# junghan0611/node-replication

Measured on AMD Instinct MI355X. Metric: Mops/s whole node, NrHashMap 10% writes, 1/2/4/8 GPUs; replay HBM GB/s vs peak, higher is better.
Workload: dtype u64; 1 GPU; NrHashMap replica per GPU: 2^26-slot table, uniform keys over 10000000, prefill [0,8388608)->k+1, rounds of 1000000 ops/GPU = 100000 Put + 900000 Get; ops_per_gpu_per_round=1000000, put_responses=Ok(None) as benches/hashmap.rs:114-119, parallelism=replicas1

## Files before the change

### include/nrgpu_testing.h

```cpp
#ifndef NRGPU_TESTING_H
#define NRGPU_TESTING_H
#include "nrgpu.h"
#ifdef __cplusplus
extern "C" {
#endif
int nrg_test_sort_pairs(nrg_ctx* ctx, const uint32_t* d_keys, const uint32_t* d_vals, uint64_t n,
                        int key_bits, uint32_t* d_out_keys, uint32_t* d_out_vals);
int nrg_test_maxscan(nrg_ctx* ctx, const uint32_t* d_keys, const uint32_t* d_vals, uint64_t n,
                     uint32_t* d_out);
int nrg_test_lds_add_order(nrg_ctx* ctx, uint32_t keys, uint32_t trials, uint32_t blocks, uint64_t out[2]);
int nrg_test_ring_read(nrg_ctx* ctx, uint64_t phys, void* out);
int nrg_test_debug_read(nrg_ctx* ctx, uint64_t* out, uint64_t words);
int nrg_test_vspace_table(nrg_ctx* ctx, uint64_t table, uint64_t out[512]);
#define NRG_MF_PREAD_TILE 16384u

#define NRG_KNOB_STAMP_MAX 1
#define NRG_KNOB_SKEW_EVERY 2
#define NRG_KNOB_EPOCH_LIMIT 3
#define NRG_KNOB_K1 4
#define NRG_KNOB_EXP 6
#define NRG_KNOB_SY_SORT 7
#define NRG_KNOB_PIPELINE 8
#define NRG_KNOB_SY_FUSED 18
#define NRG_KNOB_COMB_SPIN 10
#define NRG_KNOB_COMB_DEPTH 11
#define NRG_KNOB_PA_TPB 16
#define NRG_KNOB_COMB_GATHER 15
#define NRG_KNOB_COMB_SERVE 17
#define NRG_KNOB_SMALL_MAX 12
#define NRG_KNOB_PART 13
#define NRG_KNOB_STALL 14
#define NRG_KNOB_SL_DELTA_MAX 20
int nrg_test_set_knob(nrg_ctx* ctx, int knob, uint64_t value);
int nrg_test_combiner_probe(nrg_combiner* m, uint64_t out[8]);
int nrg_test_combiner_times(nrg_combiner* m, uint64_t out[4]);

int nrg_test_loopback_collectives(int on);
int nrg_test_hm_skewed(nrg_ctx* ctx, int* out);
#ifdef __cplusplus
}
#endif
#endif
```

### node-replication_amd/csrc/hashmap.hip

```cpp
#include <cstring>

#include "internal.hpp"
#include "../../include/nrgpu_testing.h"

namespace nrg {

typedef u64 u64x2 __attribute__((ext_vector_type(2)));

template <typename T>
__device__ __forceinline__ void st_out(T* p, T v, bool plain) {
    if (plain) *p = v;
    else __builtin_nontemporal_store(v, p);
}
__device__ __forceinline__ void st_rec(nrg_put* p, const nrg_put& r, bool plain) {
    if (plain) *p = r;
    else __builtin_nontemporal_store(u64x2{r.key, r.val}, (u64x2*)p);
}

constexpr u64 PA_NT_MAX = 2000000;
template <bool NT, typename T>
__device__ __forceinline__ void st_pol(T* p, T v) {
    if constexpr (NT) __builtin_nontemporal_store(v, p);
    else *p = v;
}
// ... 308 lines not shown
#pragma unroll
    for (int q = 0; q < K1; q++) {
        const u64 i = base + (u64)q * TPB + threadIdx.x;
        if (i >= j.n) continue;
        const u64 k = rec[q].key;
        if (k == EMPTY_KEY) {
            if (ld_relaxed32(&ctl->sp_claim) == 0 && atomicCAS(&ctl->sp_claim, 0u, 1u) == 0u) {
                ctl->sp.st[(e - 1) & 1] = stamp_make(e, 0);
                created++;
            }
            atomicMax(&s_side, (u32)(i + 1));
            j.put_slot[i] = SIDE_SLOT;
            continue;
        }
        const long long s = find_or_claim_marked(table, k, home[q], tmask, key0[q], e, &created);
        if (s < 0) {
            atomicOr(&ctl->err, ERR_TABLE_FULL);
            j.put_slot[i] = FULL_SLOT;
            continue;
        }
        j.put_slot[i] = (u32)s;
        u32 h = (u32)(mix64((u64)s) & (HT - 1));
        for (;;) {
            const u32 old = atomicCAS(&s_slot[h], 0xFFFFFFFFu, (u32)s);
            if (old == 0xFFFFFFFFu || old == (u32)s) {
                dup += old == (u32)s ? 1u : 0u;
                break;
            }
            h = (h + 1) & (HT - 1);
        }
        atomicMax(&s_max[h], (u32)(i + 1));
    }
    if (created) atomicAdd(&s_created, created);
    if (dup) atomicAdd(&s_dup, dup);
    __syncthreads();
    for (int q = threadIdx.x; q < HT; q += TPB) {
        const u32 sl = s_slot[q];
        if (sl != 0xFFFFFFFFu) {
            const u64 mine = stamp_make(e, s_max[q]);
            const u64 old = atomicMax((unsigned long long*)&table[sl].st[par], (unsigned long long)mine);
            if (old < mine) {
                j.win[s_max[q] - 1] = e;
                if (stamp_epoch(old) == e && (u32)old) j.over[(u32)old - 1] = e;
            }
        }
    }
    if (threadIdx.x == 0) {
        if (s_side) atomicMax((unsigned long long*)&ctl->sp.st[par], (unsigned long long)stamp_make(e, s_side));
        if (s_created) atomicAdd(&j.created_acc[blk % HM_CREATED_SLOTS], (u64)s_created);
        if (s_dup && j.dup_acc) atomicAdd(&j.dup_acc[blk % HM_DUP_SLOTS], (u64)s_dup);
    }
}

__device__ __forceinline__ void apply_role(const ApplyJob& j, u32 blk, Slot* table, DevCtl* ctl) {
    const u64 i = (u64)blk * TPB + threadIdx.x;
    if (i >= j.n) return;
    const u32 par = j.epoch & 1;
    const u32 s = j.put_slot[i];
    const u64 want = stamp_make(j.epoch, i + 1);
    if (s == SIDE_SLOT) {
        if (ctl->sp.st[par] == want) ctl->sp.val = j.rec.at(i).val;
    } else if (s != FULL_SLOT) {
        if (j.win[i] == j.epoch && j.over[i] != j.epoch) __builtin_nontemporal_store(j.rec.at(i).val, &table[s].val);
    }
}

__device__ __forceinline__ bool resolve(u64 val, u64 st, const ReadJob& j, u64* v) {
    const u32 se = stamp_epoch(st);
    if (st == 0 || se > j.epoch) return false;
    *v = (se == j.epoch && j.use_rec) ? j.rec.at((u32)st - 1).val : val;
    return true;
}

constexpr int RPT = 1;
static_assert(RPT == 1, "read_role gives a wave 64 consecutive Gets");

__device__ __forceinline__ u32 quad_x1(u32 x) { return (u32)__builtin_amdgcn_update_dpp(0, (int)x, 0xB1, 0xF, 0xF, true); }
__device__ __forceinline__ u32 quad_x2(u32 x) { return (u32)__builtin_amdgcn_update_dpp(0, (int)x, 0x4E, 0xF, 0xF, true); }
__device__ __forceinline__ u64 quad_or(u64 x) {
    u32 lo = (u32)x, hi = (u32)(x >> 32);
    lo |= quad_x1(lo);
    hi |= quad_x1(hi);
    lo |= quad_x2(lo);
    hi |= quad_x2(hi);
    return ((u64)hi << 32) | lo;
}

constexpr int READ_PASSES = 4;
static_assert(READ_PASSES * 16 == 64, "a wave's passes of 16 quads cover its 64 Gets");
template <bool STAMP>
__device__ __forceinline__ void read_role(const ReadJob& j, u32 blk, const Slot* table, u32 shift, u64 tmask,
                                          const DevCtl* ctl) {
    const u32 par = j.epoch & 1;
    const auto quiet = [&] { return STAMP ? false : j.quiet; };
    const auto plain = [&] { return STAMP ? true : j.plain; };
    const u32 lane = lane_id(), sub = lane & 3, quad = lane >> 2, qsh = lane & ~3u;
    const u64 wbase = (u64)blk * TPB + (threadIdx.x & ~63u);
    if (wbase >= j.R) return;
    u64 k[READ_PASSES], s[READ_PASSES], st[READ_PASSES];
    u64x2 w[READ_PASSES];
#pragma unroll
    for (int p = 0; p < READ_PASSES; p++) {
        const u64 q = wbase + p * 16 + quad;
        k[p] = q < j.R ? j.keys[q] : EMPTY_KEY;
    }
#pragma unroll
// ... 14 lines not shown
        asm volatile("" : "+v"(kk), "+v"(vv), "+v"(stt));
        bool f = false, act = k[p] != EMPTY_KEY;
        for (u64 g = 0;; g++) {
            const bool hit = act && kk == k[p];
            if (hit) {
                if (quiet()) {
                    f = true;
                    v = vv;
                } else {
                    f = resolve(vv, stt, j, &v);
                }
            }
            const u64 done = __ballot(hit || !act || kk == EMPTY_KEY);
            act = ((done >> qsh) & 15) == 0 && g < (tmask >> 2);
            if (!__ballot(act)) break;
            if (act) {
                sl = (sl + 4) & tmask;
                const u64x2 x = *(const u64x2*)&table[sl];
                if (!quiet()) stt = table[sl].st[par];
                kk = x.x;
                vv = x.y;
            }
        }
        if (k[p] == EMPTY_KEY && sub == 0 && ctl->sp_claim) {
            if (quiet()) {
                f = true;
                v = ctl->sp.val;
            } else {
                f = resolve(ctl->sp.val, ctl->sp.st[par], j, &v);
            }
        }
        if (!f) v = 0;
        rv[p] = quad_or(v);
        fb[p] = __ballot(f);
    }
    u64 c = rv[0], b = fb[0];
#pragma unroll
    for (int p = 1; p < READ_PASSES; p++) {
        if (sub == (u32)p) c = rv[p];
        if ((lane >> 4) == (u32)p) b = fb[p];
    }
    const u64 v = __shfl(c, (int)(4 * (lane & 15) + (lane >> 4)), 64);
    const u64 q = wbase + lane;
    if (q < j.R) {
        st_out(&j.vals[q], v, plain());
        st_out(&j.found[q], (uint8_t)(((b >> (4 * (lane & 15))) & 15) != 0), plain());
    }
}

constexpr int IX_STAMP = 2;
constexpr int IX_PART = 3;
constexpr int IX_PART_ALL = 4;
constexpr int IX_PART_NODUP = 5;

template <int K1, int IX>
__global__ __launch_bounds__(TPB) __attribute__((amdgpu_num_sgpr(80))) void hm_round_kernel(IndexJob ij, StampJob sj,
                                                                                             ApplyJob aj, ReadJob rj,
                                                       Slot* table, u32 shift, u64 tmask, DevCtl* ctl) {
    extern __shared__ __attribute__((aligned(16))) char s_lds[];
    u32 b = blockIdx.x;
    if (rj.s_seq && b == gridDim.x - 1) {
        if (rj.s_seq && threadIdx.x < HM_DUP_SLOTS) {
            u64 v = atomicExch((unsigned long long*)&rj.s_acc[threadIdx.x], 0ull);
#pragma unroll
            for (int off = 32; off > 0; off >>= 1) v += __shfl_xor(v, off, 64);
            if (threadIdx.x == 0) {
                rj.s_host[1] = v;
                __threadfence_system();
                rj.s_host[0] = rj.s_seq;
            }
        }
        return;
    }
    const u32 nix = IX == IX_STAMP ? sj.nblocks : ij.nblocks;
    if (b < nix) {
        if constexpr (IX == IX_STAMP) stamp_index_role<K1>(sj, b, table, shift, tmask, ctl, s_lds);
        else part_role<K1, IX == IX_PART>(ij, b, shift, s_lds);
        return;
    }
    b -= nix;
    if (b < aj.nblocks) {
        apply_role(aj, b, table, ctl);
        return;
    }
    b -= aj.nblocks;
    read_role<IX == IX_STAMP>(rj, b, table, shift, tmask, ctl);
}

struct PApplyJob {
    const u64x2* ent;
    const u32* eidx;
    const u32* cnt;
    u32 ntiles, tile, nb;
    Slot* table;
    u32 shift;
    u64 tmask;
    DevCtl* ctl;
    u64* created_acc;
    u64 lo, resp_lo, resp_hi;
    u64* prev;
    uint8_t* prevf;
    u32 stall;
    u64* dbg;
};

template <bool PREV, int T>
struct PaGeo {
    static_assert(!PREV || T == 256, "previous values use 256-thread workgroups");
    static constexpr int TPB = T;
    static constexpr int C = PREV ? 512 : 4 * T;
    static constexpr int HT = 2 * C;
    static constexpr int PER = C / TPB;
    static constexpr u32 NB_LOG = T == 1024 ? 8 : T == 512 ? 9 : 10;
};

__device__ __forceinline__ u32 pa_hash(u64 k, u32 ht) { return (u32)(mix64(k) >> 40) & (ht - 1); }

template <int N, bool WANT_VAL>
__device__ __forceinline__ void pa_resolve(Slot* table, u32 shift, u64 tmask, const u64* k, const bool* on,
                                           long long* slot, bool* fresh, u64* val) {
    u64 s[N], kk[N], vv[N];
    u32 st[N];
#pragma unroll
    for (int r = 0; r < N; r++) {
        st[r] = on[r] ? 1u : 0u;
        s[r] = on[r] ? table_home(k[r], shift) : 0;
        slot[r] = -1;
        fresh[r] = false;
        kk[r] = EMPTY_KEY;
        vv[r] = 0;
        if (on[r]) {
            if (WANT_VAL) {
                const u64x2 x = *(const u64x2*)&table[s[r]];
                kk[r] = x.x;
                vv[r] = x.y;
            } else {
                kk[r] = ld_relaxed(&table[s[r]].key);
            }
        }
// ... 986 lines not shown
            ctl->sp.st[0] = ctl->sp.st[1] = STAMP_PRESENT;
            continue;
        }
        bool fresh;
        const long long s = claim_slot(table, r.x, table_home(r.x, shift), tmask, &fresh);
        if (s < 0) {
            atomicOr(&ctl->err, ERR_TABLE_FULL);
            continue;
        }
        table[s].val = r.y;
        table[s].st[0] = table[s].st[1] = STAMP_PRESENT;
        inserted += fresh;
    }
    if (inserted) atomicAdd(&s_ins, inserted);
    __syncthreads();
    if (threadIdx.x == 0 && s_ins) atomicAdd((unsigned long long*)&ctl->nkeys, (unsigned long long)s_ins);
}

struct SegArgs {
    u64 start[64];
    u64 total;
    u32 nseg;
    u32 words;
};

__global__ __launch_bounds__(TPB) void copy_segments_kernel(const u64* __restrict__ base, u64 seg_stride_words,
                                                            SegArgs a, u64* ring, u64 ring_mask, u64 dst_lo) {
    for (u64 r = blockIdx.x * (u64)TPB + threadIdx.x; r < a.total; r += (u64)gridDim.x * TPB) {
        u32 s = 0;
        while (s + 1 < a.nseg && a.start[s + 1] <= r) s++;
        const u64 j = r - a.start[s];
        const u64* srcp = base + s * seg_stride_words + j * a.words;
        u64* dst = ring + ((dst_lo + r) & ring_mask) * a.words;
        for (u32 q = 0; q < a.words; q++) dst[q] = srcp[q];
    }
}

static inline unsigned grid_for(u64 n, u64 cap = 4096) {
    u64 g = (n + TPB - 1) / TPB;
    if (g < 1) g = 1;
    if (g > cap) g = cap;
    return (unsigned)g;
}

static RecSrc ring_src(nrg_ctx* c, const nrg_put* src, u64 lo) {
    RecSrc r;
    r.src = src;
    r.ring = (const nrg_put*)c->d_ring;
    r.mask = c->log_size - 1;
    r.lo = lo;
    return r;
}

static u32 stamp_k1_for(const nrg_ctx* c, u64 n, u64 R) {
    if (c->hm.k1_items) return c->hm.k1_items >= 4 ? 4u : c->hm.k1_items >= 2 ? 2u : 1u;
    if (n <= (1u << 18)) return 1u;
    return n >= 655360 && R >= n ? 4u : 2u;
}

struct Launch {
    IndexJob ij{};
    StampJob sj{};
    ApplyJob aj{};
    ReadJob rj{};
    int ix = IX_PART_NODUP;
    u32 K1 = 1;
    u32 nb = 0;
};

static void attach_deferred(nrg_ctx* c, Launch& L) {
    const HmDeferred& p = c->hm.pend;
    L.rj.epoch = c->hm.epoch;
    if (p.valid) {
        const RecSrc rs = ring_src(c, p.src, p.lo);
        L.rj.keys = p.keys;
        L.rj.R = p.R;
        L.rj.vals = p.vals;
        L.rj.found = p.found;
        L.rj.epoch = p.epoch;
        L.rj.use_rec = p.apply;
        L.rj.rec = rs;
        if (p.apply) {
            L.aj.rec = rs;
            L.aj.n = p.n;
            L.aj.put_slot = c->hm.d_put_slot[p.epoch & 1];
            L.aj.win = L.aj.put_slot + c->hm.stamp_alloc;
            L.aj.over = L.aj.put_slot + 2 * c->hm.stamp_alloc;
            L.aj.epoch = p.epoch;
            L.aj.nblocks = (u32)((p.n + TPB - 1) / TPB);
        }
    }
    c->hm.pend = HmDeferred{};
}

template <int K1, int IX>
static void launch_round(nrg_ctx* c, const Launch& L, u32 blocks, unsigned lds) {
    NRG_LAUNCH(c, "hm_round", (hm_round_kernel<K1, IX>), blocks, TPB, lds, c->stream, L.ij, L.sj, L.aj, L.rj,
               c->hm.d_table, c->hm.slot_shift, (u64)(c->hm.slots - 1), c->d_ctl);
}

static hipError_t launch(nrg_ctx* c, Launch& L) {
    L.rj.nblocks = (u32)((L.rj.R + TPB * RPT - 1) / (TPB * RPT));
    const u32 nix = L.ix == IX_STAMP ? L.sj.nblocks : L.ij.nblocks;
    L.ij.plain = L.sj.plain = L.rj.plain = L.ix == IX_STAMP && nix;
    L.rj.quiet = (L.ix != IX_STAMP || nix == 0) && L.aj.nblocks == 0;
    u32 blocks = nix + L.aj.nblocks + L.rj.nblocks;
    if (blocks == 0) return hipSuccess;
    if (c->hm.sample_seq) {
        L.rj.s_acc = c->hm.d_dup + ((c->hm.dup_seq - 1) & 1) * HM_DUP_SLOTS;
        L.rj.s_host = c->hm.h_dup_dev;
        L.rj.s_seq = c->hm.sample_seq;
        c->hm.sample_seq = 0;
        blocks++;
    }
    unsigned lds = 0;
    if (nix && L.ix == IX_STAMP) {
        lds = L.K1 == 4 ? StampLds<4>::BYTES : L.K1 == 2 ? StampLds<2>::BYTES : StampLds<1>::BYTES;
    } else if (nix) {
        const bool dedup = L.ix == IX_PART;
        lds = L.K1 == 8   ? PartLds<8>::bytes(dedup, L.nb)
              : L.K1 == 4 ? PartLds<4>::bytes(dedup, L.nb)
              : L.K1 == 2 ? PartLds<2>::bytes(dedup, L.nb)
                          : PartLds<1>::bytes(dedup, L.nb);
    }
    if (!nix) launch_round<1, IX_PART_NODUP>(c, L, blocks, 0);
#define NRG_RK(KK, XX) else if (L.K1 == KK && L.ix == XX) launch_round<KK, XX>(c, L, blocks, lds)
    NRG_RK(1, IX_STAMP); NRG_RK(2, IX_STAMP); NRG_RK(4, IX_STAMP);
    NRG_RK(1, IX_PART); NRG_RK(1, IX_PART_ALL); NRG_RK(1, IX_PART_NODUP);
    NRG_RK(2, IX_PART); NRG_RK(2, IX_PART_ALL); NRG_RK(2, IX_PART_NODUP);
    NRG_RK(4, IX_PART); NRG_RK(4, IX_PART_ALL); NRG_RK(4, IX_PART_NODUP);
    NRG_RK(8, IX_PART); NRG_RK(8, IX_PART_ALL); NRG_RK(8, IX_PART_NODUP);
#undef NRG_RK
    else return hipErrorInvalidValue;
    return hipGetLastError();
}

static hipError_t hm_flush(nrg_ctx* c) {
    if (!c->hm.pend.valid) return hipSuccess;
    Launch L;
    attach_deferred(c, L);
    return launch(c, L);
}

static hipError_t hm_reads(nrg_ctx* c, const u64* keys, u64 R, u64* vals, uint8_t* found) {
    if (R == 0) return hipSuccess;
    if (c->hm.pend.valid && c->hm.pend.R == 0) {
        c->hm.pend.keys = keys;
        c->hm.pend.R = R;
        c->hm.pend.vals = vals;
        c->hm.pend.found = found;
        return hm_flush(c);
    }
    hipError_t e = hm_flush(c);
    if (e != hipSuccess) return e;
    Launch L;
    attach_deferred(c, L);
    L.rj.keys = keys;
    L.rj.R = R;
    L.rj.vals = vals;
    L.rj.found = found;
    return launch(c, L);
}

static hipError_t hm_alloc(nrg_ctx* c, u64 mb) {
    const u64 tiles = (mb + TPB - 1) / TPB;
    const u64 ents = tiles * TPB;
    hipError_t e;
    if ((e = hipMalloc(&c->hm.d_bk_ent, ents * 16)) != hipSuccess) return e;
    if ((e = hipMalloc(&c->hm.d_bk_idx, ents * 4)) != hipSuccess) return e;
    if ((e = hipMalloc(&c->hm.d_bk_cnt, (u64)HM_BK_MAX * tiles * sizeof(u32))) != hipSuccess) return e;
    if (c->hm.stamp_max > mb) c->hm.stamp_max = mb;
    for (int i = 0; i < 2 && c->hm.stamp_max; i++) {
        if ((e = hipMalloc(&c->hm.d_put_slot[i], 3 * c->hm.stamp_max * sizeof(u32))) != hipSuccess) return e;
        if ((e = hipMemsetAsync(c->hm.d_put_slot[i], 0, 3 * c->hm.stamp_max * sizeof(u32), c->stream)) != hipSuccess) return e;
    }
    if ((e = hipMalloc(&c->hm.d_dup, 2 * HM_DUP_SLOTS * sizeof(u64))) != hipSuccess) return e;
    if ((e = hipMemsetAsync(c->hm.d_dup, 0, 2 * HM_DUP_SLOTS * sizeof(u64), c->stream)) != hipSuccess) return e;
    void* h = nullptr;
    if ((e = hipHostMalloc(&h, 2 * sizeof(u64), hipHostMallocMapped)) != hipSuccess) return e;
    c->hm.h_dup = (volatile u64*)h;
    c->hm.h_dup[0] = c->hm.h_dup[1] = 0;
    void* dp = nullptr;
    if ((e = hipHostGetDevicePointer(&dp, h, 0)) != hipSuccess) return e;
    c->hm.h_dup_dev = (u64*)dp;
    return hipSuccess;
}

static void hm_close(nrg_ctx* c) {
    void* ptrs[] = {c->hm.d_table, c->hm.d_created, c->hm.d_bk_ent, c->hm.d_bk_idx, c->hm.d_bk_cnt, c->hm.d_put_slot[0],
                    c->hm.d_put_slot[1], c->hm.d_dup};
    for (void* p : ptrs) (void)hipFree(p);
    if (c->hm.h_dup) (void)hipHostFree((void*)c->hm.h_dup);
    pt_close(c);
}

static hipError_t skew_sample(nrg_ctx* c) {
    if (c->hm.dup_seq && c->hm.h_dup[0] == c->hm.dup_seq && c->hm.dup_puts_sampled)
        c->hm.skewed = c->hm.h_dup[1] * 64 > c->hm.dup_puts_sampled;
    c->hm.sample_seq = ++c->hm.dup_seq;
    c->hm.dup_puts_sampled = c->hm.dup_puts;
    c->hm.dup_puts = 0;
    c->hm.dup_rounds = 0;
    return hipSuccess;
}

static int hm_open(nrg_ctx* c) {
    const nrg_config& cf = c->cfg;
    if (cf.log2_slots < 4 || cf.log2_slots > 30 || cf.max_batch > HM_MAX_BATCH) return NRG_E_INVAL;
    c->hm.grow_max_log2 = cf.hashmap_max_log2_slots;
    c->hm.slots = 1ull << cf.log2_slots;
    c->hm.slot_shift = 64 - cf.log2_slots;
    HIPCHK(hipMalloc(&c->hm.d_table, c->hm.slots * sizeof(Slot)));
    hm_init_table_kernel<<<grid_for(c->hm.slots, 16384), TPB, 0, c->stream>>>(c->hm.d_table, c->hm.slots);
    HIPCHK(hipGetLastError());
    HIPCHK(hipMalloc(&c->hm.d_created, HM_CREATED_SLOTS * sizeof(u64)));
    HIPCHK(hipMemsetAsync(c->hm.d_created, 0, HM_CREATED_SLOTS * sizeof(u64), c->stream));
    c->hm.stamp_max = HM_MAX_BATCH;
    HIPCHK(hm_alloc(c, cf.max_batch));
    c->hm.stamp_alloc = c->hm.stamp_max;
    c->pipeline = cf.pipeline != 0;
    return NRG_OK;
}

static u32 hm_slots_for(u64 keys) {
    u32 l = 4;
    while (l < 63 && (1ull << l) / HM_GROW_SLOTS_PER_KEY < keys) l++;
    return l;
}

static hipError_t hm_grow(nrg_ctx* c, u32 new_log2) {
    if (new_log2 > 30 || (1ull << new_log2) <= c->hm.slots) return hipErrorInvalidValue;
    hipError_t e = hm_flush(c);
    if (e != hipSuccess) return e;
    const u64 nslots = 1ull << new_log2;
    Slot* nt = nullptr;
    if ((e = hipMalloc(&nt, nslots * sizeof(Slot))) != hipSuccess) {
        (void)hipGetLastError();
        return hipErrorOutOfMemory;
    }
    NRG_LAUNCH(c, "hm_grow_init", hm_init_table_kernel, grid_for(nslots, 16384), TPB, 0, c->stream, nt, nslots);
    if ((e = hipGetLastError()) == hipSuccess) e = hipMemsetAsync(&c->d_ctl->nkeys, 0, sizeof(u64), c->stream);
    if (e == hipSuccess) {
        const unsigned grid = (unsigned)((c->hm.slots + RH_RUN - 1) / RH_RUN);
        NRG_LAUNCH(c, "hm_rehash", hm_rehash_kernel, grid, RH_TPB, 0, c->stream, c->hm.d_table, c->hm.slots, nt,
                   64 - new_log2, nslots - 1, c->d_ctl);
        e = hipGetLastError();
    }
    if (e == hipSuccess) e = hipMemsetAsync(c->hm.d_created, 0, HM_CREATED_SLOTS * sizeof(u64), c->stream);
    for (int i = 0; i < 2 && c->hm.d_put_slot[i] && e == hipSuccess; i++)
        e = hipMemsetAsync(c->hm.d_put_slot[i], 0, 3 * c->hm.stamp_alloc * sizeof(u32), c->stream);
    const hipError_t es = hipStreamSynchronize(c->stream);
// ... 85 lines not shown
        u32 nb_log = 0;
        while ((64ull << nb_log) < n && (1u << nb_log) < HM_BK_MAX) nb_log++;
        constexpr u64 PA_WIDE_MIN = 1ull << 16;
        const u32 pa_t = want_prev ? 256u : c->hm.pa_tpb ? c->hm.pa_tpb : n >= PA_WIDE_MIN ? 512u : 256u;
        const u32 pa_nb_log = pa_t == 1024 ? PaGeo<false, 1024>::NB_LOG : pa_t == 512 ? PaGeo<false, 512>::NB_LOG
                                                                                      : PaGeo<false, 256>::NB_LOG;
        if (nb_log > pa_nb_log) nb_log = pa_nb_log;
        if (nb_log > log2_slots) nb_log = log2_slots;
        L.ix = want_prev ? IX_PART_ALL : (c->hm.skewed || c->hm.dup_rounds + 1 >= c->hm.dup_every) ? IX_PART : IX_PART_NODUP;
        measured = L.ix == IX_PART;
        L.K1 = K1;
        L.nb = 1u << nb_log;
        IndexJob& ij = L.ij;
        ij.rec = ring_src(c, src, lo);
        ij.ring_out = write_ring ? (nrg_put*)c->d_ring : nullptr;
        ij.n = n;
        ij.nblocks = (u32)((n + tile - 1) / tile);
        ij.nb_log = nb_log;
        ij.bk_shift = log2_slots - nb_log;
        ij.ent = (u64x2*)c->hm.d_bk_ent;
        ij.eidx = want_prev ? c->hm.d_bk_idx : nullptr;
        ij.cnt = c->hm.d_bk_cnt;
        ij.dup_acc = c->hm.d_dup + (c->hm.dup_seq & 1) * HM_DUP_SLOTS;
        attach_deferred(c, L);
        if ((e = launch(c, L)) != hipSuccess) return e;
        PApplyJob aj{};
        aj.ent = ij.ent;
        aj.eidx = ij.eidx;
        aj.cnt = ij.cnt;
        aj.ntiles = ij.nblocks;
        aj.tile = tile;
        aj.nb = 1u << nb_log;
        aj.table = c->hm.d_table;
        aj.shift = c->hm.slot_shift;
        aj.tmask = c->hm.slots - 1;
        aj.ctl = c->d_ctl;
        aj.created_acc = c->hm.d_created;
        aj.lo = lo;
        aj.resp_lo = resp_lo;
        aj.resp_hi = resp_hi;
        aj.prev = d_prev;
        aj.prevf = d_prev_found;
        aj.stall = c->stall;
        aj.dbg = (c->exp & 2) ? c->d_dbg : nullptr;
        const unsigned dyn = ((ij.nblocks + 1) * 4 + ij.nblocks * 2 + 3) & ~3u;
        if (want_prev) NRG_LAUNCH(c, "hm_papply", (hm_papply_kernel<true, 256>), 1u << nb_log, 256, dyn, c->stream, aj);
        else if (pa_t == 1024) NRG_LAUNCH(c, "hm_papply", (hm_papply_kernel<false, 1024>), 1u << nb_log, 1024, dyn, c->stream, aj);
        else if (pa_t == 512 && n <= PA_NT_MAX)
            NRG_LAUNCH(c, "hm_papply", (hm_papply_kernel<false, 512, true>), 1u << nb_log, 512, dyn, c->stream, aj);
        else if (pa_t == 512) NRG_LAUNCH(c, "hm_papply", (hm_papply_kernel<false, 512>), 1u << nb_log, 512, dyn, c->stream, aj);
        else NRG_LAUNCH(c, "hm_papply", (hm_papply_kernel<false, 256>), 1u << nb_log, 256, dyn, c->stream, aj);
        if ((e = hipGetLastError()) != hipSuccess) return e;
    } else if (stamp) {
        const u32 K1 = stamp_k1_for(c, n, R);
        const u32 tile = TPB * K1;
        L.ix = IX_STAMP;
        L.K1 = K1;
        measured = true;
        L.sj.rec = ring_src(c, src, lo);
        L.sj.ring_out = write_ring ? (nrg_put*)c->d_ring : nullptr;
        L.sj.n = n;
        L.sj.nblocks = (u32)((n + tile - 1) / tile);
        L.sj.epoch = epoch;
        L.sj.put_slot = c->hm.d_put_slot[epoch & 1];
        L.sj.win = L.sj.put_slot + c->hm.stamp_alloc;
        L.sj.over = L.sj.put_slot + 2 * c->hm.stamp_alloc;
        L.sj.created_acc = c->hm.d_created;
        L.sj.dup_acc = c->hm.d_dup + (c->hm.dup_seq & 1) * HM_DUP_SLOTS;
        attach_deferred(c, L);
        if ((e = launch(c, L)) != hipSuccess) return e;
    }
    c->rounds++;
    if (measured) c->hm.dup_puts += n;
    if (++c->hm.dup_rounds >= c->hm.dup_every && (e = skew_sample(c)) != hipSuccess) return e;
    HmDeferred& p = c->hm.pend;
    p.valid = true;
    p.epoch = epoch;
    p.apply = stamp;
    p.src = keep;
    p.lo = lo;
    p.n = n;
    p.keys = d_get_keys;
    p.R = R;
    p.vals = d_get_vals;
    p.found = d_get_found;
    if (!c->pipeline || (stamp && keep)) return hm_flush(c);
    return hipSuccess;
}

static hipError_t hm_get_only(nrg_ctx* c, const u64* d_keys, u64 n, u64* d_vals, uint8_t* d_found) {
    return hm_reads(c, d_keys, n, d_vals, d_found);
}

static hipError_t hm_replay(nrg_ctx* c, const void* src, u64 lo, u64 n, u64 resp_lo, u64 resp_hi, void* d_resp,
                            uint8_t* d_some) {
    return hm_replay_chunk(c, src, lo, n, src != nullptr, nullptr, 0, nullptr, nullptr, resp_lo, resp_hi,
                           (u64*)d_resp, d_some);
}

static u64 hm_floor(const nrg_ctx* c) {
    const HmDeferred& p = c->hm.pend;
    if (p.valid && p.apply && !p.src && p.lo < c->ltail) return p.lo;
    return c->ltail;
}

static int hm_set_knob(nrg_ctx* c, int knob, uint64_t v) {
    switch (knob) {
        case NRG_KNOB_STAMP_MAX:
            c->hm.stamp_max = std::min<uint64_t>(v, c->hm.stamp_alloc);
            return NRG_OK;
        case NRG_KNOB_SKEW_EVERY:
            if (v < 1 || v > (1u << 30)) return NRG_E_INVAL;
            c->hm.dup_every = (uint32_t)v;
            return NRG_OK;
        case NRG_KNOB_EPOCH_LIMIT:
            if (v < 2 || v > 0xFFFFFFF0ull) return NRG_E_INVAL;
            c->hm.epoch_limit = (uint32_t)v;
            return NRG_OK;
        case NRG_KNOB_K1:
            if (v > 4) return NRG_E_INVAL;
            c->hm.k1_items = (uint32_t)v;
            return NRG_OK;
        case NRG_KNOB_PART:
            if (v > 2) return NRG_E_INVAL;
            c->hm.part_mode = (uint32_t)v;
            return NRG_OK;
        case NRG_KNOB_PA_TPB:
            if (v != 0 && v != 256 && v != 512 && v != 1024) return NRG_E_INVAL;
            c->hm.pa_tpb = (uint32_t)v;
            return NRG_OK;
        case NRG_KNOB_SMALL_MAX:
            if (v > 2048) return NRG_E_INVAL;
            c->hm.small_max = v;
            return NRG_OK;
        default: return NRG_E_INVAL;
    }
}

static u64 hm_dbg_words(const nrg_ctx*) { return (u64)HM_BK_MAX * 8; }

static hipError_t hm_digest(nrg_ctx* c, u64* d_out3);
static int hm_items(nrg_ctx* c, u64* n);
static hipError_t hm_snapshot(nrg_ctx* c, void* d_buf, u64 cap, u64 log_idx);
static int hm_restore(nrg_ctx* c, const void* d_payload, u64 items, bool check_only);

const DsOps* hm_ops() {
    static const DsOps ops = {sizeof(nrg_put), sizeof(u64), hm_open, hm_close, hm_flush, hm_replay,
                              hm_floor, hm_set_knob, hm_dbg_words, nullptr, hm_digest,
                              hm_items, hm_snapshot, hm_restore};
    return &ops;
}

hipError_t hm_prefill_range(nrg_ctx* c, u64 n, u64 off, u32 part, u32 parts) {
    hipError_t e = hm_flush(c);
    if (e != hipSuccess) return e;
    u64 mine = n;
    if (parts > 1 && c->hm.grow_max_log2 > 64 - c->hm.slot_shift) {
        mine = 0;
        for (u64 k = 0; k < n; k++) mine += key_owner(k, parts) == part;
    }
    if ((e = hm_room(c, mine)) != hipSuccess) return e;
    hm_prefill_range_kernel<<<grid_for(n, 8192), TPB, 0, c->stream>>>(c->hm.d_table, n, off, c->hm.slot_shift,
                                                                      c->hm.slots - 1, c->d_ctl, part, parts);
    return hipGetLastError();
}

static hipError_t hm_count(nrg_ctx* c) {
    hipError_t e = hm_flush(c);
    if (e != hipSuccess) return e;
    hm_count_kernel<<<1, TPB, 0, c->stream>>>(c->hm.d_created, HM_CREATED_SLOTS, c->d_ctl);
    return hipGetLastError();
}

static hipError_t hm_dump(nrg_ctx* c, u64* d_keys, u64* d_vals) {
    hipError_t e = hm_flush(c);
// ... 20 lines not shown
    HIPCHK(hipMemcpyAsync(n, &c->d_ctl->nkeys_total, 8, hipMemcpyDeviceToHost, c->stream));
    HIPCHK(hipStreamSynchronize(c->stream));
    return NRG_OK;
}

static hipError_t hm_snapshot(nrg_ctx* c, void* d_buf, u64 cap, u64 log_idx) {
    hipError_t e = hm_flush(c);
    if (e != hipSuccess) return e;
    if ((e = hipMemsetAsync(&c->d_ctl->counter, 0, sizeof(u64), c->stream)) != hipSuccess) return e;
    const u64 cap_items = cap >= SNAP_HDR ? (cap - SNAP_HDR) / 16 : 0;
    const u64 tiles = (c->hm.slots + SN_TILE - 1) / SN_TILE;
    NRG_LAUNCH(c, "hm_snapshot", hm_snapshot_kernel, (unsigned)(tiles < 8192 ? tiles : 8192), TPB, 0, c->stream,
               (const Slot*)c->hm.d_table, (u64)c->hm.slots, c->d_ctl, (u64x2*)((char*)d_buf + SNAP_HDR), cap_items);
    if ((e = hipGetLastError()) != hipSuccess) return e;
    hm_snapshot_head_kernel<<<1, 64, 0, c->stream>>>(c->d_ctl, (u64*)d_buf, cap, log_idx);
    return hipGetLastError();
}

static int hm_restore(nrg_ctx* c, const void* d_payload, u64 items, bool check_only) {
    const u32 cur = 64 - c->hm.slot_shift;
    const bool grows = c->hm.grow_max_log2 > cur;
    if (check_only) {
        const u64 limit = grows ? (1ull << c->hm.grow_max_log2) / HM_GROW_SLOTS_PER_KEY : c->hm.slots;
        return items > limit ? NRG_E_TABLE_FULL : NRG_OK;
    }
    if (!d_payload) items = 0;
    if (grows) {
        u32 want = hm_slots_for(items);
        if (want > c->hm.grow_max_log2) want = c->hm.grow_max_log2;
        if ((1ull << want) > c->hm.slots) {
            Slot* nt = nullptr;
            if (hipMalloc(&nt, (1ull << want) * sizeof(Slot)) != hipSuccess) {
                (void)hipGetLastError();
                return NRG_E_NOMEM;
            }
            (void)hipFree(c->hm.d_table);
            c->hm.d_table = nt;
            c->hm.slots = 1ull << want;
            c->hm.slot_shift = 64 - want;
        }
    }
    c->hm.pend.valid = false;
    NRG_LAUNCH(c, "hm_restore_init", hm_init_table_kernel, grid_for(c->hm.slots, 16384), TPB, 0, c->stream,
               c->hm.d_table, c->hm.slots);
    HIPCHK(hipGetLastError());
    HIPCHK(hipMemsetAsync(c->d_ctl, 0, sizeof(DevCtl), c->stream));
    HIPCHK(hipMemsetAsync(c->hm.d_created, 0, HM_CREATED_SLOTS * sizeof(u64), c->stream));
    for (int i = 0; i < 2 && c->hm.d_put_slot[i]; i++)
        HIPCHK(hipMemsetAsync(c->hm.d_put_slot[i], 0, 3 * c->hm.stamp_alloc * sizeof(u32), c->stream));
    HIPCHK(hipMemsetAsync(c->hm.d_dup, 0, 2 * HM_DUP_SLOTS * sizeof(u64), c->stream));
    c->hm.h_dup[0] = c->hm.h_dup[1] = 0;
    c->hm.dup_seq = c->hm.dup_puts = c->hm.dup_puts_sampled = c->hm.sample_seq = 0;
    c->hm.dup_rounds = 0;
    c->hm.skewed = false;
    c->hm.epoch = 1;
    c->hm.keys_ub = items;
    if (items) {
        NRG_LAUNCH(c, "hm_restore", hm_restore_kernel, grid_for(items, 8192), TPB, 0, c->stream, c->hm.d_table,
                   (const u64x2*)d_payload, items, c->hm.slot_shift, (u64)(c->hm.slots - 1), c->d_ctl);
        HIPCHK(hipGetLastError());
    }
    return NRG_OK;
}

hipError_t copy_segments(nrg_ctx* c, const void* d_base, u32 nseg, u64 seg_stride, const u64* lens, u64 dst_lo) {
    SegArgs a;
    if (nseg > 64) return hipErrorInvalidValue;
    a.nseg = nseg;
    a.words = c->rec_bytes / 8;
    u64 acc = 0;
    for (u32 s = 0; s < nseg; s++) {
        a.start[s] = acc;
        acc += lens[s];
    }
    a.total = acc;
    if (acc == 0) return hipSuccess;
    copy_segments_kernel<<<grid_for(acc, 8192), TPB, 0, c->stream>>>(
        (const u64*)d_base, seg_stride * a.words, a, (u64*)c->d_ring, c->log_size - 1, dst_lo);
    return hipGetLastError();
}

int hm_small_job(nrg_ctx* c, const nrg_put* recs, u64 W, u32 origin, const u64* keys, u64 R, u64* vals,
                 uint8_t* found, u64* prev, uint8_t* prevf, u32* e_out, SmallJobBlob* blob, u64* lo_out) {
    if (!c || c->cfg.ds_kind != NRG_DS_HASHMAP || W > c->cfg.max_batch || c->ltail != c->tail) return NRG_E_INVAL;
    if ((W && !recs) || (R && (!keys || !vals || !found))) return NRG_E_INVAL;
    int r = reserve(c, W);
    if (r) return r == NRG_E_RING_FULL ? NRG_E_INVAL : r;
    const uint64_t lo = c->tail;
    if (!hm_small_fill(c, recs, lo, W, keys, R, vals, found, prev, prevf, e_out, blob)) return NRG_E_INVAL;
    bool due = false;
    if (hm_room(c, W, &due) != hipSuccess || due) return NRG_E_INVAL;
    if (lo_out) *lo_out = lo;
    c->rounds++;
    if (W) note_origin(c, lo, W, origin);
    commit_round(c, lo, W);
    return NRG_OK;
}

}

using namespace nrg;

extern "C" {

int nrg_hashmap_get_async(nrg_ctx* c, const uint64_t* d_keys, uint64_t n, uint64_t* d_vals, uint8_t* d_found) {
    int r = need(c, NRG_DS_HASHMAP);
    if (r) return r;
// ... 111 lines not shown
}

int nrg_hashmap_reserve(nrg_ctx* c, uint64_t n_keys) {
    int r = need(c, NRG_DS_HASHMAP);
    if (r) return r;
    if (n_keys > (1ull << 30) / HM_GROW_SLOTS_PER_KEY) return NRG_E_INVAL;
    const uint32_t want = hm_slots_for(n_keys);
    if ((1ull << want) <= c->hm.slots) return NRG_OK;
    HIPCHK(hm_grow(c, want));
    return NRG_OK;
}

int nrg_hashmap_capacity(nrg_ctx* c, uint32_t* log2_slots) {
    if (!c || !log2_slots || c->cfg.ds_kind != NRG_DS_HASHMAP) return NRG_E_INVAL;
    *log2_slots = 64 - c->hm.slot_shift;
    return NRG_OK;
}

int nrg_hashmap_size(nrg_ctx* c, uint64_t* n) {
    int r = need(c, NRG_DS_HASHMAP);
    if (r) return r;
    HIPCHK(hm_count(c));
    HIPCHK(hipMemcpyAsync(n, &c->d_ctl->nkeys_total, 8, hipMemcpyDeviceToHost, c->stream));
    HIPCHK(sync_all(c));
    return check_err(c);
}

int nrg_hashmap_dump(nrg_ctx* c, uint64_t* keys, uint64_t* vals, uint64_t cap, uint64_t* n) {
    int r = nrg_hashmap_size(c, n);
    if (r) return r;
    if (*n > cap) return NRG_E_CAPACITY;
    if (*n == 0) return NRG_OK;
    Staging* s = c->stg;
    if ((r = staging(s[0], *n * 8)) || (r = staging(s[1], *n * 8))) return r;
    HIPCHK(hm_dump(c, (u64*)s[0].p, (u64*)s[1].p));
    HIPCHK(hipMemcpyAsync(keys, s[0].p, *n * 8, hipMemcpyDeviceToHost, c->stream));
    HIPCHK(hipMemcpyAsync(vals, s[1].p, *n * 8, hipMemcpyDeviceToHost, c->stream));
    HIPCHK(sync_all(c));
    return check_err(c);
}

int nrg_hashmap_digest(nrg_ctx* c, uint64_t out[3]) {
    int r = need(c, NRG_DS_HASHMAP);
    if (r) return r;
    return nrg_digest(c, out);
}

int nrg_test_hm_skewed(nrg_ctx* c, int* out) {
    if (!c || !out || c->cfg.ds_kind != NRG_DS_HASHMAP) return NRG_E_INVAL;
    *out = c->hm.skewed ? 1 : 0;
    return NRG_OK;
}

}
```

### node-replication_amd/csrc/internal.hpp

```cpp
#pragma once

#include <hip/hip_ext.h>
#include <hip/hip_runtime.h>
#include <stdint.h>

#include <map>
#include <string>
#include <vector>

#include "../../include/nrgpu.h"
#include "capacity.hpp"
#include "common.hpp"

namespace nrg {

struct SortScratch {
    u64 cap = 0;
    u32* k[2] = {nullptr, nullptr};
    u32* v[2] = {nullptr, nullptr};
    u32* ctlmem = nullptr;
    u64 max_tiles = 0;
    u64 ctl_words = 0;
};

// ... 49 lines not shown
    u64 rlo = 0, rhi = 0;
    u64* resp = nullptr;
    uint8_t* some = nullptr;
};

struct QuState {
    u64 head, len;
    u64 ck_head, ck_len, ck_pops;
};

struct VsState {
    u64 ntables;
};

struct SlState {
    u64 nb, nd;
    u64 nd_in, nnew;
};

struct HostRun {
    u64 first, count;
    u32 origin;
};


struct HmHost {
    uint32_t slot_shift = 0;
    uint64_t slots = 0;
    Slot* d_table = nullptr;
    uint32_t grow_max_log2 = 0;
    uint64_t keys_ub = 0;
    uint32_t k1_items = 0;
    HmDeferred pend;
    uint64_t small_max = 0;
    uint64_t* d_created = nullptr;
    void* d_bk_ent = nullptr;
    uint32_t* d_bk_idx = nullptr;
    uint32_t* d_bk_cnt = nullptr;
    uint64_t stamp_max = 0;
    uint32_t part_mode = 1;
    uint32_t pa_tpb = 0;
    uint64_t stamp_alloc = 0;
    uint32_t epoch = 1;
    uint32_t epoch_limit = 0xFFFFFFF0u;
    uint32_t* d_put_slot[2] = {nullptr, nullptr};
    uint64_t* d_dup = nullptr;
    volatile uint64_t* h_dup = nullptr;
    uint64_t* h_dup_dev = nullptr;
    uint64_t dup_seq = 0, dup_puts = 0, dup_puts_sampled = 0;
    uint64_t sample_seq = 0;
    uint32_t* err_out = nullptr;
    uint32_t dup_rounds = 0, dup_every = 16;
    bool skewed = false;
};

struct StHost {
    uint32_t* d_stack = nullptr;
    void* d_aux = nullptr;
    StDeferred pend;
    uint32_t par = 0;
    uint32_t* d_desc = nullptr;
    uint64_t desc_words = 0;
};

struct SyHost {
    uint64_t* d_words = nullptr;
    uint64_t* d_sort_aux = nullptr;
    uint32_t key_bits = 0;
    void* d_aux = nullptr;
    SyDeferred pend;
    SyDeferred pend_b;
    bool fused = true;
    uint32_t round = 0;
    uint64_t* d_tmp = nullptr;
    uint32_t* d_desc = nullptr;
    uint64_t desc_words = 0;
};

struct QuHost {
    uint64_t* d_queue = nullptr;
    uint64_t size = 0;
    QuState* d_state = nullptr;
    void* d_aux = nullptr;
};

struct VsHost {
    uint64_t* d_pool = nullptr;
    uint64_t cap = 0;
    VsState* d_state = nullptr;
    void* d_aux = nullptr;
    uint64_t* d_tag = nullptr;
};

struct SlHost {
    uint64_t* d_bk[2] = {nullptr, nullptr};
    uint64_t* d_bv[2] = {nullptr, nullptr};
    uint64_t* d_dk[2] = {nullptr, nullptr};
    uint64_t* d_dv[2] = {nullptr, nullptr};
    uint32_t bcur = 0, dcur = 0;
    uint64_t cap = 0;
    uint64_t delta_max = 0;
    uint64_t dcap = 0;
    SlState* d_state = nullptr;
    uint64_t *d_sk = nullptr, *d_nk = nullptr, *d_nv = nullptr;
    uint32_t *d_sp = nullptr, *d_k32 = nullptr, *d_pv = nullptr, *d_tcnt = nullptr;
    uint8_t* d_miss = nullptr;
// ... 229 lines not shown
```

### node-replication_amd/nrgpu/_lib.py

```python
from __future__ import annotations

import ctypes as C
import os

import numpy as np

_HERE = os.path.dirname(os.path.abspath(__file__))
PKG_ROOT = os.path.dirname(_HERE)
LIB_PATH = os.environ.get("NRGPU_LIB") or os.path.join(PKG_ROOT, "lib", "libnrgpu.so")

try:
    import torch
except Exception:
    torch = None

NRG_OK = 0
NRG_E_INVAL = -1
NRG_E_HIP = -2
NRG_E_TABLE_FULL = -3
NRG_E_RING_FULL = -4
NRG_E_NOMEM = -5
NRG_E_NOT_SYNCED = -6
NRG_E_CAPACITY = -7
NRG_E_NODEV = -8
# ... 268 lines not shown
    "nrg_gen_zipf_async": (C.c_int, [vp, vp, u64, u64, u64, C.c_double, C.c_int]),
    "nrg_gen_stack_ops_async": (C.c_int, [vp, vp, u64, u64]),
    "nrg_kernel_timing": (C.c_int, [vp, C.c_int]),
    "nrg_kernel_timing_only": (C.c_int, [vp, C.c_char_p]),
    "nrg_kernel_time": (C.c_int, [vp, C.c_char_p, u64p, C.POINTER(C.c_double)]),
    "nrg_group_unique_id": (C.c_int, [vp]),
    "nrg_group_join": (C.c_int, [vp, vp, C.c_int, C.c_int, C.POINTER(vp)]),
    "nrg_group_open": (C.c_int, [C.POINTER(C.c_int), C.c_int, C.POINTER(Config), C.POINTER(vp)]),
    "nrg_group_close": (C.c_int, [vp]),
    "nrg_group_info": (C.c_int, [vp, C.POINTER(C.c_int), C.POINTER(C.c_int), C.POINTER(C.c_int)]),
    "nrg_group_replica": (vp, [vp, C.c_int]),
    "nrg_group_set_input_stream": (C.c_int, [vp, C.c_int, vp]),
    "nrg_group_round_async": (C.c_int, [vp, C.POINTER(Round), u64p]),
    "nrg_group_sync": (C.c_int, [vp]),
    "nrg_group_set_timeout": (C.c_int, [vp, u32]),
    "nrg_group_last_error": (C.c_char_p, [vp]),
    "nrg_combiner_open": (C.c_int, [vp, u32, C.POINTER(vp)]),
    "nrg_combiner_close": (C.c_int, [vp]),
    "nrg_combiner_register": (C.c_int, [vp, C.POINTER(u32)]),
    "nrg_combiner_put": (C.c_int, [vp, u32, vp, vp, u32, vp, vp]),
    "nrg_combiner_execute_mut": (C.c_int, [vp, u32, vp, u32, vp, vp]),
    "nrg_combiner_execute": (C.c_int, [vp, u32, vp, u32, vp, vp]),
    "nrg_combiner_get": (C.c_int, [vp, u32, vp, u32, vp, vp]),
    "nrg_combiner_stats": (C.c_int, [vp, u64p, u64p]),
    "nrg_key_owner": (C.c_uint32, [u64, C.c_uint32]),
    "nrg_hashmap_partition_async": (C.c_int, [vp, vp, u64, vp, u64, C.c_uint32, vp, vp, vp, vp, vp]),
    "nrg_route_back_async": (C.c_int, [vp, vp, vp, vp, u64, vp, vp]),
    "nrg_hashmap_prefill_partition": (C.c_int, [vp, u64, u64, C.c_uint32, C.c_uint32]),
    "nrg_group_partitioned_round": (C.c_int, [vp, C.POINTER(Round)]),
    "nrg_group_partitioned_round_async": (C.c_int, [vp, C.POINTER(Round)]),
    "nrg_group_partitioned_flush": (C.c_int, [vp]),
    "nrg_memfs_owner": (C.c_uint32, [u64, C.c_uint32]),
    "nrg_memfs_partition_async": (C.c_int, [vp, vp, u64, C.c_uint32, vp, vp, vp]),
    "nrg_memfs_route_back_async": (C.c_int, [vp, vp, vp, vp, u64, vp, vp]),
    "nrg_group_file_round": (C.c_int, [vp, C.POINTER(Round)]),
    "nrg_memfs_rd_partition_async": (C.c_int, [vp, vp, u64, C.c_uint32, vp, vp, vp]),
    "nrg_memfs_pread_repack_async": (C.c_int, [vp, vp, vp, vp, vp, u64, vp, u64, vp, vp]),
    "nrg_group_memfs_pread": (C.c_int, [vp, C.POINTER(Pread)]),
    "nrg_group_skiplist_seek": (C.c_int, [vp, C.POINTER(Seek), C.c_uint32]),
    "nrg_group_skiplist_range_count": (C.c_int, [vp, C.POINTER(Count)]),
    "nrg_group_skiplist_scan": (C.c_int, [vp, C.POINTER(Scan), C.c_uint32, C.c_uint32]),
}

TEST_SIGNATURES = {
    "nrg_test_combiner_probe": (C.c_int, [vp, C.POINTER(C.c_uint64)]),
    "nrg_test_combiner_times": (C.c_int, [vp, C.POINTER(C.c_uint64)]),
    "nrg_test_sort_pairs": (C.c_int, [vp, vp, vp, u64, C.c_int, vp, vp]),
    "nrg_test_maxscan": (C.c_int, [vp, vp, vp, u64, vp]),
    "nrg_test_lds_add_order": (C.c_int, [vp, u32, u32, u32, vp]),
    "nrg_test_ring_read": (C.c_int, [vp, u64, vp]),
    "nrg_test_debug_read": (C.c_int, [vp, vp, u64]),
    "nrg_test_vspace_table": (C.c_int, [vp, u64, vp]),
    "nrg_test_hm_skewed": (C.c_int, [vp, vp]),
    "nrg_test_set_knob": (C.c_int, [vp, C.c_int, u64]),
    "nrg_test_loopback_collectives": (C.c_int, [C.c_int]),
}

KNOBS = {"STAMP_MAX": 1, "SKEW_EVERY": 2, "EPOCH_LIMIT": 3, "K1": 4, "EXP": 6, "SY_SORT": 7,
         "PIPELINE": 8, "COMB_SPIN": 10, "COMB_DEPTH": 11,
         "SMALL_MAX": 12, "PART": 13, "STALL": 14, "COMB_GATHER": 15, "PA_TPB": 16, "COMB_SERVE": 17, "SY_FUSED": 18,
         "SL_DELTA_MAX": 20}

_lib = None


def load(path: str = LIB_PATH):
    global _lib
    if _lib is None:
        if not os.path.exists(path):
            raise OSError(f"libnrgpu.so not built at {path}: run `make -C node-replication_amd` "
                          "(or __graft_entry__.build()); there is no CPU fallback")
        L = C.CDLL(path)
        for name, (res, args) in {**SIGNATURES, **TEST_SIGNATURES}.items():
            f = getattr(L, name)
            f.restype = res
            f.argtypes = args
        _lib = L
    return _lib


def check(code: int, what: str = ""):
    if code != NRG_OK:
        raise NrgError(code, what)
    return code


def default_config(kind: int) -> Config:
    cfg = Config()
    load().nrg_config_default(C.byref(cfg), kind)
    return cfg
```

Measured before the change: 31670 Mops/s.

## Add direct per-put atomic-max winner election path for hashmap stamp indexing

Measured after the change: 31670 Mops/s, median of 2. No clear change (-0.0%).

```diff
diff --git a/include/nrgpu_testing.h b/include/nrgpu_testing.h
--- a/include/nrgpu_testing.h
+++ b/include/nrgpu_testing.h
@@ -18,6 +18,7 @@
 #define NRG_KNOB_SKEW_EVERY 2
 #define NRG_KNOB_EPOCH_LIMIT 3
 #define NRG_KNOB_K1 4
+#define NRG_KNOB_HM_ELECT 21
 #define NRG_KNOB_EXP 6
 #define NRG_KNOB_SY_SORT 7
 #define NRG_KNOB_PIPELINE 8
@@ -37,6 +38,7 @@
 
 int nrg_test_loopback_collectives(int on);
 int nrg_test_hm_skewed(nrg_ctx* ctx, int* out);
+int nrg_test_hm_index_rounds(nrg_ctx* ctx, uint64_t out[2]);
 #ifdef __cplusplus
 }
 #endif
diff --git a/node-replication_amd/csrc/hashmap.hip b/node-replication_amd/csrc/hashmap.hip
--- a/node-replication_amd/csrc/hashmap.hip
+++ b/node-replication_amd/csrc/hashmap.hip
@@ -384,6 +384,83 @@
     }
 }
 
+template <int K1>
+__device__ __forceinline__ void stamp_elect_role(const StampJob& j, u32 blk, Slot* table, u32 shift, u64 tmask,
+                                                 DevCtl* ctl) {
+    constexpr int TILE = TPB * K1;
+    const u32 e = j.epoch, par = e & 1;
+    const u64 base = (u64)blk * TILE;
+    nrg_put rec[K1];
+    u64 home[K1], key0[K1];
+#pragma unroll
+    for (int q = 0; q < K1; q++) {
+        const u64 i = base + (u64)q * TPB + threadIdx.x;
+        rec[q] = i < j.n ? j.rec.at(i) : nrg_put{EMPTY_KEY, 0};
+    }
+#pragma unroll
+    for (int q = 0; q < K1; q++) {
+        const u64 i = base + (u64)q * TPB + threadIdx.x;
+        if (i < j.n && j.ring_out) st_rec(&j.ring_out[(j.rec.lo + i) & j.rec.mask], rec[q], j.plain);
+        home[q] = table_home(rec[q].key, shift);
+        key0[q] = i < j.n && rec[q].key != EMPTY_KEY ? table[home[q]].key : EMPTY_KEY;
+    }
+    u64* stp[K1];
+    u32 created = 0;
+#pragma unroll
+    for (int q = 0; q < K1; q++) {
+        const u64 i = base + (u64)q * TPB + threadIdx.x;
+        stp[q] = nullptr;
+        if (i >= j.n) continue;
+        const u64 k = rec[q].key;
+        if (k == EMPTY_KEY) {
+            if (ld_relaxed32(&ctl->sp_claim) == 0 && atomicCAS(&ctl->sp_claim, 0u, 1u) == 0u) {
+                ctl->sp.st[(e - 1) & 1] = stamp_make(e, 0);
+                created++;
+            }
+            j.put_slot[i] = SIDE_SLOT;
+            stp[q] = &ctl->sp.st[par];
+            continue;
+        }
+        const long long s = find_or_claim_marked(table, k, home[q], tmask, key0[q], e, &created);
+        if (s < 0) {
+            atomicOr(&ctl->err, ERR_TABLE_FULL);
+            j.put_slot[i] = FULL_SLOT;
+            continue;
+        }
+        j.put_slot[i] = (u32)s;
+        stp[q] = &table[s].st[par];
+    }
+    u64 old[K1];
+#pragma unroll
+    for (int q = 0; q < K1; q++) {
+        const u64 i = base + (u64)q * TPB + threadIdx.x;
+        old[q] = ~0ull;
+        typedef __attribute__((address_space(1))) unsigned long long gu64;
+        if (stp[q])
+            old[q] = __hip_atomic_fetch_max((gu64*)stp[q], (unsigned long long)stamp_make(e, i + 1), __ATOMIC_RELAXED,
+                                            __HIP_MEMORY_SCOPE_AGENT);
+    }
+    u32 dup = 0;
+#pragma unroll
+    for (int q = 0; q < K1; q++) {
+        const u64 i = base + (u64)q * TPB + threadIdx.x;
+        if (!stp[q]) continue;
+        if (old[q] < stamp_make(e, i + 1)) {
+            j.win[i] = e;
+            if (stamp_epoch(old[q]) == e && (u32)old[q]) j.over[(u32)old[q] - 1] = e;
+        }
+        dup += stamp_epoch(old[q]) == e ? 1u : 0u;
+    }
+    u32 both = created | (dup << 16);
+#pragma unroll
+    for (int off = 32; off > 0; off >>= 1) both += __shfl_xor(both, off, 64);
+    if ((threadIdx.x & 63) == 0 && both) {
+        const u32 w = blk * (TPB / 64) + (threadIdx.x >> 6);
+        if (both & 0xFFFFu) atomicAdd(&j.created_acc[w % HM_CREATED_SLOTS], (u64)(both & 0xFFFFu));
+        if ((both >> 16) && j.dup_acc) atomicAdd(&j.dup_acc[w % HM_DUP_SLOTS], (u64)(both >> 16));
+    }
+}
+
 __device__ __forceinline__ void apply_role(const ApplyJob& j, u32 blk, Slot* table, DevCtl* ctl) {
     const u64 i = (u64)blk * TPB + threadIdx.x;
     if (i >= j.n) return;
@@ -504,6 +581,19 @@
 constexpr int IX_PART = 3;
 constexpr int IX_PART_ALL = 4;
 constexpr int IX_PART_NODUP = 5;
+constexpr int IX_ELECT = 6;
+
+#ifdef NRG_HM_ROLE_MARKS
+constexpr u64 HM_MARK_WAVES = 1ull << 16;
+__device__ u64* g_hm_marks;
+#define HM_MARK(WORD)                                                                               \
+    do {                                                                                            \
+        const u64 gw_ = (u64)blockIdx.x * (TPB / 64) + (threadIdx.x >> 6);                          \
+        if ((threadIdx.x & 63) == 0 && g_hm_marks && gw_ < HM_MARK_WAVES) g_hm_marks[2 * gw_ + (WORD)] = wall_clock64(); \
+    } while (0)
+#else
+#define HM_MARK(WORD) ((void)0)
+#endif
 
 template <int K1, int IX>
 __global__ __launch_bounds__(TPB) __attribute__((amdgpu_num_sgpr(80))) void hm_round_kernel(IndexJob ij, StampJob sj,
@@ -524,19 +614,25 @@
         }
         return;
     }
-    const u32 nix = IX == IX_STAMP ? sj.nblocks : ij.nblocks;
+    constexpr bool STAMP = IX == IX_STAMP || IX == IX_ELECT;
+    const u32 nix = STAMP ? sj.nblocks : ij.nblocks;
+    HM_MARK(0);
     if (b < nix) {
         if constexpr (IX == IX_STAMP) stamp_index_role<K1>(sj, b, table, shift, tmask, ctl, s_lds);
+        else if constexpr (IX == IX_ELECT) stamp_elect_role<K1>(sj, b, table, shift, tmask, ctl);
         else part_role<K1, IX == IX_PART>(ij, b, shift, s_lds);
+        HM_MARK(1);
         return;
     }
     b -= nix;
     if (b < aj.nblocks) {
         apply_role(aj, b, table, ctl);
+        HM_MARK(1);
         return;
     }
     b -= aj.nblocks;
-    read_role<IX == IX_STAMP>(rj, b, table, shift, tmask, ctl);
+    read_role<STAMP>(rj, b, table, shift, tmask, ctl);
+    HM_MARK(1);
 }
 
 struct PApplyJob {
@@ -1629,10 +1725,19 @@
     return r;
 }
 
-static u32 stamp_k1_for(const nrg_ctx* c, u64 n, u64 R) {
+constexpr u64 ELECT_SMALL_MAX = 100000;
+constexpr u64 ELECT_K2_MIN = 175000;
+static u32 stamp_k1_for(const nrg_ctx* c, u64 n, u64 R, bool direct) {
     if (c->hm.k1_items) return c->hm.k1_items >= 4 ? 4u : c->hm.k1_items >= 2 ? 2u : 1u;
-    if (n <= (1u << 18)) return 1u;
+    if (direct) {
+        if (n < ELECT_K2_MIN) return 1u;
+    } else if (n <= (1u << 18)) return 1u;
     return n >= 655360 && R >= n ? 4u : 2u;
+}
+
+static bool stamp_direct_for(const nrg_ctx* c, u64 n) {
+    if (c->hm.elect_mode) return c->hm.elect_mode == 2;
+    return c->hm.sampled && !c->hm.skewed && (n <= ELECT_SMALL_MAX || n >= ELECT_K2_MIN);
 }
 
 struct Launch {
@@ -1678,9 +1783,10 @@
 
 static hipError_t launch(nrg_ctx* c, Launch& L) {
     L.rj.nblocks = (u32)((L.rj.R + TPB * RPT - 1) / (TPB * RPT));
-    const u32 nix = L.ix == IX_STAMP ? L.sj.nblocks : L.ij.nblocks;
-    L.ij.plain = L.sj.plain = L.rj.plain = L.ix == IX_STAMP && nix;
-    L.rj.quiet = (L.ix != IX_STAMP || nix == 0) && L.aj.nblocks == 0;
+    const bool stamp = L.ix == IX_STAMP || L.ix == IX_ELECT;
+    const u32 nix = stamp ? L.sj.nblocks : L.ij.nblocks;
+    L.ij.plain = L.sj.plain = L.rj.plain = stamp && nix;
+    L.rj.quiet = (!stamp || nix == 0) && L.aj.nblocks == 0;
     u32 blocks = nix + L.aj.nblocks + L.rj.nblocks;
     if (blocks == 0) return hipSuccess;
     if (c->hm.sample_seq) {
@@ -1693,6 +1799,8 @@
     unsigned lds = 0;
     if (nix && L.ix == IX_STAMP) {
         lds = L.K1 == 4 ? StampLds<4>::BYTES : L.K1 == 2 ? StampLds<2>::BYTES : StampLds<1>::BYTES;
+    } else if (nix && L.ix == IX_ELECT) {
+        lds = 0;
     } else if (nix) {
         const bool dedup = L.ix == IX_PART;
         lds = L.K1 == 8   ? PartLds<8>::bytes(dedup, L.nb)
@@ -1703,6 +1811,7 @@
     if (!nix) launch_round<1, IX_PART_NODUP>(c, L, blocks, 0);
 #define NRG_RK(KK, XX) else if (L.K1 == KK && L.ix == XX) launch_round<KK, XX>(c, L, blocks, lds)
     NRG_RK(1, IX_STAMP); NRG_RK(2, IX_STAMP); NRG_RK(4, IX_STAMP);
+    NRG_RK(1, IX_ELECT); NRG_RK(2, IX_ELECT); NRG_RK(4, IX_ELECT);
     NRG_RK(1, IX_PART); NRG_RK(1, IX_PART_ALL); NRG_RK(1, IX_PART_NODUP);
     NRG_RK(2, IX_PART); NRG_RK(2, IX_PART_ALL); NRG_RK(2, IX_PART_NODUP);
     NRG_RK(4, IX_PART); NRG_RK(4, IX_PART_ALL); NRG_RK(4, IX_PART_NODUP);
@@ -1772,8 +1881,10 @@
 }
 
 static hipError_t skew_sample(nrg_ctx* c) {
-    if (c->hm.dup_seq && c->hm.h_dup[0] == c->hm.dup_seq && c->hm.dup_puts_sampled)
+    if (c->hm.dup_seq && c->hm.h_dup[0] == c->hm.dup_seq && c->hm.dup_puts_sampled) {
         c->hm.skewed = c->hm.h_dup[1] * 64 > c->hm.dup_puts_sampled;
+        c->hm.sampled = true;
+    }
     c->hm.sample_seq = ++c->hm.dup_seq;
     c->hm.dup_puts_sampled = c->hm.dup_puts;
     c->hm.dup_puts = 0;
@@ -1965,9 +2076,11 @@
         else NRG_LAUNCH(c, "hm_papply", (hm_papply_kernel<false, 256>), 1u << nb_log, 256, dyn, c->stream, aj);
         if ((e = hipGetLastError()) != hipSuccess) return e;
     } else if (stamp) {
-        const u32 K1 = stamp_k1_for(c, n, R);
+        const bool direct = stamp_direct_for(c, n);
+        const u32 K1 = stamp_k1_for(c, n, R, direct);
         const u32 tile = TPB * K1;
-        L.ix = IX_STAMP;
+        L.ix = direct ? IX_ELECT : IX_STAMP;
+        c->hm.index_rounds[direct ? 1 : 0]++;
         L.K1 = K1;
         measured = true;
         L.sj.rec = ring_src(c, src, lo);
@@ -2034,6 +2147,10 @@
             if (v > 4) return NRG_E_INVAL;
             c->hm.k1_items = (uint32_t)v;
             return NRG_OK;
+        case NRG_KNOB_HM_ELECT:
+            if (v > 2) return NRG_E_INVAL;
+            c->hm.elect_mode = (uint32_t)v;
+            return NRG_OK;
         case NRG_KNOB_PART:
             if (v > 2) return NRG_E_INVAL;
             c->hm.part_mode = (uint32_t)v;
@@ -2160,7 +2277,7 @@
     c->hm.h_dup[0] = c->hm.h_dup[1] = 0;
     c->hm.dup_seq = c->hm.dup_puts = c->hm.dup_puts_sampled = c->hm.sample_seq = 0;
     c->hm.dup_rounds = 0;
-    c->hm.skewed = false;
+    c->hm.skewed = c->hm.sampled = false;
     c->hm.epoch = 1;
     c->hm.keys_ub = items;
     if (items) {
@@ -2378,4 +2495,26 @@
     return NRG_OK;
 }
 
-}
+int nrg_test_hm_index_rounds(nrg_ctx* c, uint64_t out[2]) {
+    if (!c || !out || c->cfg.ds_kind != NRG_DS_HASHMAP) return NRG_E_INVAL;
+    out[0] = c->hm.index_rounds[0];
+    out[1] = c->hm.index_rounds[1];
+    return NRG_OK;
+}
+
+#ifdef NRG_HM_ROLE_MARKS
+int nrg_diag_hm_marks(uint64_t* out, uint64_t words) {
+    static uint64_t* d_marks = nullptr;
+    if (words > 2 * nrg::HM_MARK_WAVES) return NRG_E_INVAL;
+    if (hipDeviceSynchronize() != hipSuccess) return NRG_E_HIP;
+    if (!d_marks) {
+        if (hipMalloc(&d_marks, 2 * nrg::HM_MARK_WAVES * sizeof(uint64_t)) != hipSuccess) return NRG_E_HIP;
+        if (hipMemcpyToSymbol(HIP_SYMBOL(nrg::g_hm_marks), &d_marks, sizeof(d_marks)) != hipSuccess) return NRG_E_HIP;
+    } else if (out && hipMemcpy(out, d_marks, words * sizeof(uint64_t), hipMemcpyDeviceToHost) != hipSuccess) {
+        return NRG_E_HIP;
+    }
+    return hipMemset(d_marks, 0, 2 * nrg::HM_MARK_WAVES * sizeof(uint64_t)) == hipSuccess ? NRG_OK : NRG_E_HIP;
+}
+#endif
+
+}
diff --git a/node-replication_amd/csrc/internal.hpp b/node-replication_amd/csrc/internal.hpp
--- a/node-replication_amd/csrc/internal.hpp
+++ b/node-replication_amd/csrc/internal.hpp
@@ -125,6 +125,9 @@
     uint32_t* err_out = nullptr;
     uint32_t dup_rounds = 0, dup_every = 16;
     bool skewed = false;
+    bool sampled = false;
+    uint32_t elect_mode = 0;
+    uint64_t index_rounds[2] = {0, 0};
 };
 
 struct StHost {
diff --git a/node-replication_amd/nrgpu/_lib.py b/node-replication_amd/nrgpu/_lib.py
--- a/node-replication_amd/nrgpu/_lib.py
+++ b/node-replication_amd/nrgpu/_lib.py
@@ -344,6 +344,7 @@
     "nrg_test_debug_read": (C.c_int, [vp, vp, u64]),
     "nrg_test_vspace_table": (C.c_int, [vp, u64, vp]),
     "nrg_test_hm_skewed": (C.c_int, [vp, vp]),
+    "nrg_test_hm_index_rounds": (C.c_int, [vp, C.POINTER(C.c_uint64)]),
     "nrg_test_set_knob": (C.c_int, [vp, C.c_int, u64]),
     "nrg_test_loopback_collectives": (C.c_int, [C.c_int]),
 }
@@ -351,7 +352,7 @@
 KNOBS = {"STAMP_MAX": 1, "SKEW_EVERY": 2, "EPOCH_LIMIT": 3, "K1": 4, "EXP": 6, "SY_SORT": 7,
          "PIPELINE": 8, "COMB_SPIN": 10, "COMB_DEPTH": 11,
          "SMALL_MAX": 12, "PART": 13, "STALL": 14, "COMB_GATHER": 15, "PA_TPB": 16, "COMB_SERVE": 17, "SY_FUSED": 18,
-         "SL_DELTA_MAX": 20}
+         "SL_DELTA_MAX": 20, "HM_ELECT": 21}
 
 _lib = None
 
```
